# sonbui25/Multimodal-Aspect-Category-Sentiment-Analysis

Measured on AMD Instinct MI355X. Metric: train samples/sec (fwd+bwd+step) FCMF seq128x36ROI, higher is better.
Workload: dtype bf16; 1 GPU; FCMF-base fine-tune step, BASELINE configs[1]: batch 64 reviews x 6 aspects per GPU, seq 128, 7 images x (49 patches + 36 ROIs), precomputed ResNet-152 features, dropout 0.1, clip 1.0 + 4-group AdamW + linear schedule; global_batch=64, per_gpu_batch=64, seq_len=128, parallelism=dp1, sample_unit=1 review = 6 aspect forwards

## Files before the change

multimodal-aspect-category-sentiment-analysis_amd/csrc/misc.hip:

```cpp
#include "common.h"

template <typename T>
__global__ __launch_bounds__(256) void xent_fwd_kernel(const T* __restrict__ logits, int64_t ld,
                                                       const int64_t* __restrict__ labels, float* __restrict__ loss_rows,
                                                       float* __restrict__ nvalid, int n, int C, int64_t ignore_index) {
  const int lane = threadIdx.x & 63;
  const int row = blockIdx.x * 4 + (threadIdx.x >> 6);
  if (row >= n) return;
  const int64_t lab = labels[row];
  if (lab == ignore_index) { if (lane == 0) loss_rows[row] = 0.f; return; }
  const T* lr = logits + (int64_t)row * ld;
  float m = -INFINITY;
  for (int c = lane; c < C; c += 64) m = fmaxf(m, to_f32<T>(lr[c]));
  m = wave_max(m);
  float s = 0.f;
  for (int c = lane; c < C; c += 64) s += __expf(to_f32<T>(lr[c]) - m);
  s = wave_sum(s);
  if (lane == 0) {
    loss_rows[row] = (m + __logf(s)) - to_f32<T>(lr[lab]);
    if (nvalid) atomicAdd(nvalid, 1.0f);
  }
}

__global__ __launch_bounds__(256) void xent_mean_kernel(const float* __restrict__ loss_rows, const int64_t* __restrict__ labels,
                                                        int n, int64_t ignore_index, float mult, float* __restrict__ out2) {
  __shared__ double ssum[256];
  __shared__ int scnt[256];
  double s = 0.0;
  int c = 0;
  for (int i = threadIdx.x; i < n; i += 256)
    if (labels[i] != ignore_index) { s += (double)loss_rows[i]; ++c; }
  ssum[threadIdx.x] = s; scnt[threadIdx.x] = c;
  __syncthreads();
  for (int h = 128; h > 0; h >>= 1) {
    if ((int)threadIdx.x < h) { ssum[threadIdx.x] += ssum[threadIdx.x + h]; scnt[threadIdx.x] += scnt[threadIdx.x + h]; }
    __syncthreads();
  }
  if (threadIdx.x == 0) {
    const float nv = (float)scnt[0];
    out2[0] = mult * ((float)ssum[0] / nv);
    out2[1] = mult / nv;
  }
}

template <typename T>
__global__ __launch_bounds__(256) void bce_logits_kernel(const T* __restrict__ logits, int64_t ld, const float* __restrict__ target,
                                                         int64_t ldt, int n, int C, const float* __restrict__ dloss,
                                                         float* __restrict__ loss, T* __restrict__ dlogits, int64_t ldd,
                                                         float* __restrict__ probs) {
  __shared__ double ssum[256];
  const int64_t total = (int64_t)n * C;
  const float sc = (dloss ? *dloss : 1.0f) / (float)total;
  double s = 0.0;
// ... 102 lines not shown
  row_softmax_stats<T>(lr, C, vec != 0, m, s);
  if (threadIdx.x == 0) {
    loss_rows[row] = (m + __logf(s)) - to_f32<T>(lr[lab]);
    if (nvalid) atomicAdd(nvalid, 1.0f);
  }
}

template <typename T>
__global__ __launch_bounds__(256) void xent_bwd_wide_kernel(const T* logits, int64_t ld, const int64_t* __restrict__ labels,
                                                            T* dlogits, int64_t ldd, const float* __restrict__ scale_ptr,
                                                            float extra, int C, int64_t ignore_index, int vec) {
  constexpr int VN = XVec<T>::N;
  typedef typename XVec<T>::type vec_t;
  const int row = blockIdx.x, tid = threadIdx.x;
  const int64_t lab = labels[row];
  T* dr = dlogits + (int64_t)row * ldd;
  const int Cv = vec ? (C / VN) * VN : 0;
  if (lab == ignore_index) {
    vec_t z;
#pragma unroll
    for (int e = 0; e < VN; ++e) z[e] = from_f32<T>(0.f);
    for (int c = tid * VN; c < Cv; c += 256 * VN) *reinterpret_cast<vec_t*>(dr + c) = z;
    for (int c = Cv + tid; c < C; c += 256) dr[c] = from_f32<T>(0.f);
    return;
  }
  const T* lr = logits + (int64_t)row * ld;
  float m, s;
  row_softmax_stats<T>(lr, C, vec != 0, m, s);
  const float sc = (scale_ptr ? *scale_ptr : 1.0f) * extra, inv = sc / s;
  for (int c = tid * VN; c < Cv; c += 256 * VN) {
    const vec_t v = *reinterpret_cast<const vec_t*>(lr + c);
    vec_t o;
#pragma unroll
    for (int e = 0; e < VN; ++e) o[e] = from_f32<T>(__expf((float)v[e] - m) * inv - ((c + e) == lab ? sc : 0.f));
    *reinterpret_cast<vec_t*>(dr + c) = o;
  }
  for (int c = Cv + tid; c < C; c += 256) dr[c] = from_f32<T>(__expf(to_f32<T>(lr[c]) - m) * inv - (c == lab ? sc : 0.f));
}

template <typename TS, typename TD>
__global__ __launch_bounds__(256) void cast_kernel(const TS* __restrict__ s, TD* __restrict__ d, int64_t n) {
  const int64_t n4 = n >> 2;
  for (int64_t i = (int64_t)blockIdx.x * 256 + threadIdx.x; i < n4; i += (int64_t)gridDim.x * 256)
    Vec4<TD>::store(d + i * 4, Vec4<TS>::load(s + i * 4));
  if (blockIdx.x == 0 && threadIdx.x < (n & 3)) d[n4 * 4 + threadIdx.x] = from_f32<TD>(to_f32<TS>(s[n4 * 4 + threadIdx.x]));
}

template <typename TS, typename TD>
__global__ __launch_bounds__(256) void cast_unaligned_kernel(const TS* __restrict__ s, TD* __restrict__ d, int64_t n) {
  for (int64_t i = (int64_t)blockIdx.x * 256 + threadIdx.x; i < n; i += (int64_t)gridDim.x * 256)
    d[i] = from_f32<TD>(to_f32<TS>(s[i]));
}

__global__ __launch_bounds__(256) void cast_transpose_kernel(const float* __restrict__ src, bf16_t* __restrict__ dst, int R, int C) {
  __shared__ float tile[64][65];
  const int r0 = blockIdx.y * 64, c0 = blockIdx.x * 64;
  const int tx = threadIdx.x & 63, ty = threadIdx.x >> 6;
#pragma unroll
  for (int i = 0; i < 16; ++i) {
    const int r = r0 + ty * 16 + i, c = c0 + tx;
    tile[ty * 16 + i][tx] = (r < R && c < C) ? src[(int64_t)r * C + c] : 0.f;
  }
  __syncthreads();
  if ((R & 3) == 0) {
#pragma unroll
    for (int i = 0; i < 4; ++i) {
      const int cc = i * 16 + (threadIdx.x >> 4), rr = 4 * (threadIdx.x & 15);
      const int c = c0 + cc, r = r0 + rr;
      if (c < C && r < R) {
        bf16x4 o;
#pragma unroll
        for (int j = 0; j < 4; ++j) o[j] = (bf16_t)tile[rr + j][cc];
        *reinterpret_cast<bf16x4*>(dst + (int64_t)c * R + r) = o;
      }
    }
    return;
  }
#pragma unroll
  for (int i = 0; i < 16; ++i) {
    const int c = c0 + ty * 16 + i, r = r0 + tx;
    if (c < C && r < R) dst[(int64_t)c * R + r] = (bf16_t)tile[tx][ty * 16 + i];
  }
}

__global__ __launch_bounds__(256) void multi_cast_transpose_kernel(const int64_t* __restrict__ src_ptrs, const int64_t* __restrict__ dst_ptrs,
                                                                   const int32_t* __restrict__ dims, const int32_t* __restrict__ desc) {
  __shared__ float tile[64][65];
  const int t = desc[3 * blockIdx.x], r0 = desc[3 * blockIdx.x + 1] * 64, c0 = desc[3 * blockIdx.x + 2] * 64;
  const float* __restrict__ src = reinterpret_cast<const float*>(src_ptrs[t]);
  bf16_t* __restrict__ dst = reinterpret_cast<bf16_t*>(dst_ptrs[t]);
  const int R = dims[2 * t], C = dims[2 * t + 1];
  const int tx = threadIdx.x & 63, ty = threadIdx.x >> 6;
#pragma unroll
  for (int i = 0; i < 16; ++i) {
    const int r = r0 + ty * 16 + i, c = c0 + tx;
    tile[ty * 16 + i][tx] = (r < R && c < C) ? src[(int64_t)r * C + c] : 0.f;
  }
  __syncthreads();
#pragma unroll
  for (int i = 0; i < 16; ++i) {
    const int c = c0 + ty * 16 + i, r = r0 + tx;
    if (c < C && r < R) dst[(int64_t)c * R + r] = (bf16_t)tile[tx][ty * 16 + i];
  }
}

template <typename T>
__global__ __launch_bounds__(256) void dropout_kernel(const T* __restrict__ x, T* __restrict__ y, int64_t n, float p,
                                                      float inv_keep, uint64_t seed) {
  for (int64_t i = (int64_t)blockIdx.x * 256 + threadIdx.x; i < n; i += (int64_t)gridDim.x * 256)
    y[i] = from_f32<T>(to_f32<T>(x[i]) * dropout_mult(seed, (uint64_t)i, p, inv_keep));
}

template <typename T>
__global__ __launch_bounds__(256) void act_bwd_kernel(const T* __restrict__ dy, const T* __restrict__ aux, T* __restrict__ out,
                                                      int64_t n, int kind) {
  for (int64_t i = (int64_t)blockIdx.x * 256 + threadIdx.x; i < n; i += (int64_t)gridDim.x * 256) {
    const float a = to_f32<T>(aux[i]), d = to_f32<T>(dy[i]);
    out[i] = from_f32<T>(kind == 0 ? d * (1.0f - a * a) : d * dgelu_f(a));
  }
}

template <typename T>
__global__ __launch_bounds__(256) void sum_axis_kernel(const T* __restrict__ in, T* __restrict__ out, int64_t outer,
                                                       int reps, int64_t inner) {
  const int64_t total = outer * inner;
  for (int64_t i = (int64_t)blockIdx.x * 256 + threadIdx.x; i < total; i += (int64_t)gridDim.x * 256) {
    const int64_t o = i / inner, c = i - o * inner;
    float s = 0.f;
    for (int r = 0; r < reps; ++r) s += to_f32<T>(in[(o * reps + r) * inner + c]);
    out[i] = from_f32<T>(s);
  }
}

__global__ __launch_bounds__(256) void multi_sumsq_kernel(const int64_t* __restrict__ g_ptrs, const int64_t* __restrict__ sizes,
                                                          const int32_t* __restrict__ chunk_tensor,
                                                          const int64_t* __restrict__ chunk_offset, int chunk_size,
                                                          double* __restrict__ sumsq, double* __restrict__ per_tensor) {
  __shared__ double red[4];
  const int t = chunk_tensor[blockIdx.x];
  const int64_t off = chunk_offset[blockIdx.x];
  const float* g = reinterpret_cast<const float*>(g_ptrs[t]) + off;
  int64_t n = sizes[t] - off;
  if (n > chunk_size) n = chunk_size;
  double s = 0.0;
  const bool vec = (reinterpret_cast<uintptr_t>(g) & 15) == 0;
  if (vec) {
    const int64_t n4 = n >> 2;
    for (int64_t i = threadIdx.x; i < n4; i += 256) {
      const float4 v = *reinterpret_cast<const float4*>(g + i * 4);
      s += (double)v.x * v.x + (double)v.y * v.y + (double)v.z * v.z + (double)v.w * v.w;
    }
    for (int64_t i = n4 * 4 + threadIdx.x; i < n; i += 256) s += (double)g[i] * g[i];
  } else {
    for (int64_t i = threadIdx.x; i < n; i += 256) s += (double)g[i] * g[i];
  }
  s = wave_sum_d(s);
  if ((threadIdx.x & 63) == 0) red[threadIdx.x >> 6] = s;
  __syncthreads();
  if (threadIdx.x == 0) {
    const double tot = red[0] + red[1] + red[2] + red[3];
    if (sumsq) atomicAdd(sumsq, tot);
    if (per_tensor) atomicAdd(per_tensor + t, tot);
  }
}

struct AdamArgs {
  const int64_t *p_ptrs, *g_ptrs, *m_ptrs, *v_ptrs, *bf16_ptrs, *sizes;
  const int32_t *group_of, *chunk_tensor;
  const int64_t* chunk_offset;
  int chunk_size;
  float lr[8], wd[8];
  float beta1, beta2, eps, bc1, bc2_sqrt;
  const double* sumsq;
  float max_norm;
};

__global__ __launch_bounds__(256) void multi_adamw_kernel(AdamArgs a) {
#pragma clang fp contract(off)
  const int t = a.chunk_tensor[blockIdx.x];
  const int64_t off = a.chunk_offset[blockIdx.x];
  float* p = reinterpret_cast<float*>(a.p_ptrs[t]) + off;
  const float* g = reinterpret_cast<const float*>(a.g_ptrs[t]) + off;
  float* m = reinterpret_cast<float*>(a.m_ptrs[t]) + off;
  float* v = reinterpret_cast<float*>(a.v_ptrs[t]) + off;
  bf16_t* sh = a.bf16_ptrs && a.bf16_ptrs[t] ? reinterpret_cast<bf16_t*>(a.bf16_ptrs[t]) + off : nullptr;
  int64_t n = a.sizes[t] - off;
  if (n > a.chunk_size) n = a.chunk_size;
  const int grp = a.group_of[t];
  const float lr = a.lr[grp], wd = a.wd[grp];
  float coef = 1.0f;
  if (a.max_norm > 0.f && a.sumsq) {
    const float tn = (float)sqrt(*a.sumsq);
    coef = fminf(1.0f, a.max_norm / (tn + 1e-6f));
  }
  const float step_size = lr / a.bc1;
  typedef float f4 __attribute__((ext_vector_type(4)));
  int64_t i0 = 0;
  if (((reinterpret_cast<uintptr_t>(p) | reinterpret_cast<uintptr_t>(g) | reinterpret_cast<uintptr_t>(m) | reinterpret_cast<uintptr_t>(v)) & 15) == 0 &&
      (!sh || (reinterpret_cast<uintptr_t>(sh) & 7) == 0)) {
    const int64_t n4 = n >> 2;
    for (int64_t i = threadIdx.x; i < n4; i += 256) {
      const f4 g4 = __builtin_nontemporal_load(reinterpret_cast<const f4*>(g) + i) * coef;
      f4 p4 = reinterpret_cast<const f4*>(p)[i] * (1.0f - lr * wd);
// ... 5 lines not shown
      __builtin_nontemporal_store(m4, reinterpret_cast<f4*>(m) + i);
      __builtin_nontemporal_store(v4, reinterpret_cast<f4*>(v) + i);
      if (sh) {
        bf16x4 o;
        o[0] = (bf16_t)p4[0]; o[1] = (bf16_t)p4[1]; o[2] = (bf16_t)p4[2]; o[3] = (bf16_t)p4[3];
        reinterpret_cast<bf16x4*>(sh)[i] = o;
      }
    }
    i0 = n4 << 2;
  }
  for (int64_t i = i0 + threadIdx.x; i < n; i += 256) {
    const float gi = g[i] * coef;
    float pi = p[i] * (1.0f - lr * wd);
    const float mi = a.beta1 * m[i] + (1.0f - a.beta1) * gi;
    const float vi = a.beta2 * v[i] + (1.0f - a.beta2) * gi * gi;
    const float denom = sqrtf(vi) / a.bc2_sqrt + a.eps;
    pi -= step_size * (mi / denom);
    p[i] = pi; m[i] = mi; v[i] = vi;
    if (sh) sh[i] = (bf16_t)pi;
  }
}

__global__ __launch_bounds__(256) void sumsq_kernel(const float* __restrict__ g, int64_t n, double* __restrict__ out) {
  __shared__ double red[4];
  double s = 0.0;
  for (int64_t i = (int64_t)blockIdx.x * 256 + threadIdx.x; i < n; i += (int64_t)gridDim.x * 256) s += (double)g[i] * g[i];
  s = wave_sum_d(s);
  if ((threadIdx.x & 63) == 0) red[threadIdx.x >> 6] = s;
  __syncthreads();
  if (threadIdx.x == 0) atomicAdd(out, red[0] + red[1] + red[2] + red[3]);
}

__global__ __launch_bounds__(256) void bertadam_kernel(float* __restrict__ p, const float* __restrict__ g, float* __restrict__ m,
                                                       float* __restrict__ v, int64_t n, float lr, float b1, float b2, float e,
                                                       float wd, float max_norm, const double* __restrict__ sumsq) {
  float coef = 1.0f;
  if (max_norm > 0.f) coef = fminf(1.0f, max_norm / ((float)sqrt(*sumsq) + 1e-6f));
  for (int64_t i = (int64_t)blockIdx.x * 256 + threadIdx.x; i < n; i += (int64_t)gridDim.x * 256) {
    const float gi = g[i] * coef;
    const float mi = b1 * m[i] + (1.0f - b1) * gi;
    const float vi = b2 * v[i] + (1.0f - b2) * gi * gi;
    float upd = mi / (sqrtf(vi) + e);
    if (wd > 0.f) upd += wd * p[i];
    p[i] -= lr * upd;
    m[i] = mi; v[i] = vi;
  }
}

static int grid_for(int64_t n, int per) {
  int64_t b = (n + per - 1) / per;
  return (int)(b > 4096 ? 4096 : (b < 1 ? 1 : b));
}

extern "C" int fcmf_abi_version(void) { return 4; }
extern "C" const char* fcmf_build_info(void) { return "libfcmf_hip gfx950 (CDNA4, wave64) abi 4"; }

extern "C" int fcmf_xent_fwd(const void* logits, int64_t ld, const int64_t* labels, float* loss_rows, float* nvalid, int n,
                             int C, int64_t ignore_index, int dtype, void* stream) {
  if (!logits || !labels || !loss_rows || n < 0 || C <= 0) return FCMF_ERR_ARG;
  if (n == 0) return FCMF_OK;
  hipStream_t st = reinterpret_cast<hipStream_t>(stream);
  if (C >= 1024) {
    const int es = dtype == FCMF_F32 ? 4 : 2;
    const int vec = ((reinterpret_cast<uintptr_t>(logits) & 15) == 0) && ((ld * es) % 16 == 0);
    if (dtype == FCMF_F32) hipLaunchKernelGGL((xent_fwd_wide_kernel<float>), dim3(n), dim3(256), 0, st, (const float*)logits, ld, labels, loss_rows, nvalid, C, ignore_index, vec);
    else if (dtype == FCMF_BF16) hipLaunchKernelGGL((xent_fwd_wide_kernel<bf16_t>), dim3(n), dim3(256), 0, st, (const bf16_t*)logits, ld, labels, loss_rows, nvalid, C, ignore_index, vec);
    else return FCMF_ERR_UNSUPPORTED;
    FCMF_CHECK_LAUNCH();
    return FCMF_OK;
  }
  dim3 grid((n + 3) / 4);
  if (dtype == FCMF_F32) hipLaunchKernelGGL((xent_fwd_kernel<float>), grid, dim3(256), 0, st, (const float*)logits, ld, labels, loss_rows, nvalid, n, C, ignore_index);
  else if (dtype == FCMF_BF16) hipLaunchKernelGGL((xent_fwd_kernel<bf16_t>), grid, dim3(256), 0, st, (const bf16_t*)logits, ld, labels, loss_rows, nvalid, n, C, ignore_index);
  else return FCMF_ERR_UNSUPPORTED;
  FCMF_CHECK_LAUNCH();
  return FCMF_OK;
}

extern "C" int fcmf_xent_mean(const float* loss_rows, const int64_t* labels, int n, int64_t ignore_index, float mult,
                              float* out2, void* stream) {
  if (!loss_rows || !labels || !out2 || n < 0) return FCMF_ERR_ARG;
  hipLaunchKernelGGL(xent_mean_kernel, dim3(1), dim3(256), 0, reinterpret_cast<hipStream_t>(stream), loss_rows, labels, n,
                     ignore_index, mult, out2);
  FCMF_CHECK_LAUNCH();
  return FCMF_OK;
}

extern "C" int fcmf_bce_logits(const void* logits, int64_t ld, const float* target, int64_t ldt, int n, int C, const float* dloss,
                               float* loss, void* dlogits, int64_t ldd, float* probs, int dtype, void* stream) {
  if (!logits || (!target && (loss || dlogits)) || n < 0 || C <= 0 || ld < C || (target && ldt < C) || (dlogits && ldd < C))
    return FCMF_ERR_ARG;
  if (n == 0) return FCMF_OK;
  hipStream_t st = reinterpret_cast<hipStream_t>(stream);
  if (dtype == FCMF_F32)
    hipLaunchKernelGGL((bce_logits_kernel<float>), dim3(1), dim3(256), 0, st, (const float*)logits, ld, target, ldt, n, C, dloss, loss,
                       (float*)dlogits, ldd, probs);
  else if (dtype == FCMF_BF16)
    hipLaunchKernelGGL((bce_logits_kernel<bf16_t>), dim3(1), dim3(256), 0, st, (const bf16_t*)logits, ld, target, ldt, n, C, dloss, loss,
                       (bf16_t*)dlogits, ldd, probs);
  else return FCMF_ERR_UNSUPPORTED;
  FCMF_CHECK_LAUNCH();
  return FCMF_OK;
}

extern "C" int fcmf_additive_mask(const int64_t* mask, int64_t ld, float* out, int rows, int cols, float value, void* stream) {
  if (!mask || !out || rows < 0 || cols < 0 || ld < cols) return FCMF_ERR_ARG;
// ... 28 lines not shown
  FCMF_CHECK_LAUNCH();
  return FCMF_OK;
}

extern "C" int fcmf_cast(const void* src, void* dst, int64_t n, int src_dtype, int dst_dtype, void* stream) {
  if (!src || !dst || n < 0) return FCMF_ERR_ARG;
  if (n == 0) return FCMF_OK;
  hipStream_t st = reinterpret_cast<hipStream_t>(stream);
  if ((reinterpret_cast<uintptr_t>(src) & 15) || (reinterpret_cast<uintptr_t>(dst) & 7)) {
    const uintptr_t sm = src_dtype == FCMF_F32 ? 3 : 1, dm = dst_dtype == FCMF_F32 ? 3 : 1;
    if ((reinterpret_cast<uintptr_t>(src) & sm) || (reinterpret_cast<uintptr_t>(dst) & dm)) return FCMF_ERR_ARG;
    dim3 g1(grid_for(n, 256));
    if (src_dtype == FCMF_F32 && dst_dtype == FCMF_BF16) hipLaunchKernelGGL((cast_unaligned_kernel<float, bf16_t>), g1, dim3(256), 0, st, (const float*)src, (bf16_t*)dst, n);
    else if (src_dtype == FCMF_BF16 && dst_dtype == FCMF_F32) hipLaunchKernelGGL((cast_unaligned_kernel<bf16_t, float>), g1, dim3(256), 0, st, (const bf16_t*)src, (float*)dst, n);
    else if (src_dtype == FCMF_F32 && dst_dtype == FCMF_F32) hipLaunchKernelGGL((cast_unaligned_kernel<float, float>), g1, dim3(256), 0, st, (const float*)src, (float*)dst, n);
    else if (src_dtype == FCMF_BF16 && dst_dtype == FCMF_BF16) hipLaunchKernelGGL((cast_unaligned_kernel<bf16_t, bf16_t>), g1, dim3(256), 0, st, (const bf16_t*)src, (bf16_t*)dst, n);
    else return FCMF_ERR_UNSUPPORTED;
    FCMF_CHECK_LAUNCH();
    return FCMF_OK;
  }
  dim3 grid(grid_for(n, 1024));
  if (src_dtype == FCMF_F32 && dst_dtype == FCMF_BF16) hipLaunchKernelGGL((cast_kernel<float, bf16_t>), grid, dim3(256), 0, st, (const float*)src, (bf16_t*)dst, n);
  else if (src_dtype == FCMF_BF16 && dst_dtype == FCMF_F32) hipLaunchKernelGGL((cast_kernel<bf16_t, float>), grid, dim3(256), 0, st, (const bf16_t*)src, (float*)dst, n);
  else if (src_dtype == FCMF_F32 && dst_dtype == FCMF_F32) hipLaunchKernelGGL((cast_kernel<float, float>), grid, dim3(256), 0, st, (const float*)src, (float*)dst, n);
  else if (src_dtype == FCMF_BF16 && dst_dtype == FCMF_BF16) hipLaunchKernelGGL((cast_kernel<bf16_t, bf16_t>), grid, dim3(256), 0, st, (const bf16_t*)src, (bf16_t*)dst, n);
  else return FCMF_ERR_UNSUPPORTED;
  FCMF_CHECK_LAUNCH();
  return FCMF_OK;
}

extern "C" int fcmf_cast_transpose(const float* src, void* dst, int rows, int cols, void* stream) {
  if (!src || !dst || rows < 0 || cols < 0) return FCMF_ERR_ARG;
  if (rows == 0 || cols == 0) return FCMF_OK;
  dim3 grid((cols + 63) / 64, (rows + 63) / 64);
  hipLaunchKernelGGL(cast_transpose_kernel, grid, dim3(256), 0, reinterpret_cast<hipStream_t>(stream), src, (bf16_t*)dst, rows, cols);
  FCMF_CHECK_LAUNCH();
  return FCMF_OK;
}

extern "C" int fcmf_multi_cast_transpose(const int64_t* src_ptrs, const int64_t* dst_ptrs, const int32_t* dims,
                                         const int32_t* tile_desc, int ntiles, void* stream) {
  if (!src_ptrs || !dst_ptrs || !dims || !tile_desc || ntiles < 0) return FCMF_ERR_ARG;
  if (ntiles == 0) return FCMF_OK;
  hipLaunchKernelGGL(multi_cast_transpose_kernel, dim3(ntiles), dim3(256), 0, reinterpret_cast<hipStream_t>(stream), src_ptrs,
                     dst_ptrs, dims, tile_desc);
  FCMF_CHECK_LAUNCH();
  return FCMF_OK;
}

extern "C" int fcmf_dropout(const void* x, void* y, int64_t n, float p, uint64_t seed, int dtype, void* stream) {
  if (!x || !y || n < 0 || p < 0.f || p >= 1.f) return FCMF_ERR_ARG;
  if (n == 0) return FCMF_OK;
  hipStream_t st = reinterpret_cast<hipStream_t>(stream);
  dim3 grid(grid_for(n, 256));
  const float inv_keep = 1.0f / (1.0f - p);
  if (dtype == FCMF_F32) hipLaunchKernelGGL((dropout_kernel<float>), grid, dim3(256), 0, st, (const float*)x, (float*)y, n, p, inv_keep, seed);
  else if (dtype == FCMF_BF16) hipLaunchKernelGGL((dropout_kernel<bf16_t>), grid, dim3(256), 0, st, (const bf16_t*)x, (bf16_t*)y, n, p, inv_keep, seed);
  else return FCMF_ERR_UNSUPPORTED;
  FCMF_CHECK_LAUNCH();
  return FCMF_OK;
}

extern "C" int fcmf_act_bwd(const void* dy, const void* aux, void* out, int64_t n, int kind, int dtype, void* stream) {
  if (!dy || !aux || !out || n < 0 || (kind != 0 && kind != 1)) return FCMF_ERR_ARG;
  if (n == 0) return FCMF_OK;
  hipStream_t st = reinterpret_cast<hipStream_t>(stream);
  dim3 grid(grid_for(n, 256));
  if (dtype == FCMF_F32) hipLaunchKernelGGL((act_bwd_kernel<float>), grid, dim3(256), 0, st, (const float*)dy, (const float*)aux, (float*)out, n, kind);
  else if (dtype == FCMF_BF16) hipLaunchKernelGGL((act_bwd_kernel<bf16_t>), grid, dim3(256), 0, st, (const bf16_t*)dy, (const bf16_t*)aux, (bf16_t*)out, n, kind);
  else return FCMF_ERR_UNSUPPORTED;
  FCMF_CHECK_LAUNCH();
  return FCMF_OK;
}

template <typename T>
__global__ __launch_bounds__(256) void embed_scale_fwd_kernel(const int64_t* __restrict__ ids, const float* __restrict__ w,
                                                              const float* __restrict__ P, T* __restrict__ out, int n, int H,
                                                              int S, float scale, int64_t V) {
  const int lane = threadIdx.x & 63, row = blockIdx.x * 4 + (threadIdx.x >> 6);
  if (row >= n) return;
  const int64_t id = ids[row];
  if (id < 0 || id >= V) {
    const float q = __builtin_nanf("");
    for (int c = lane * 4; c < H; c += 256) Vec4<T>::store(out + (int64_t)row * H + c, make_float4(q, q, q, q));
    return;
  }
  const float* wr = w + id * (int64_t)H;
  const float* pr = P ? P + (int64_t)(row % S) * H : nullptr;
  for (int c = lane * 4; c < H; c += 256) {
    float4 v = *reinterpret_cast<const float4*>(wr + c);
    v.x *= scale; v.y *= scale; v.z *= scale; v.w *= scale;
    if (pr) {
      const float4 q = *reinterpret_cast<const float4*>(pr + c);
      v.x += q.x; v.y += q.y; v.z += q.z; v.w += q.w;
    }
    Vec4<T>::store(out + (int64_t)row * H + c, v);
  }
}
template <typename T>
__global__ __launch_bounds__(256) void embed_scale_bwd_kernel(const T* __restrict__ dy, const int64_t* __restrict__ ids,
                                                              float* __restrict__ dw, int n, int H, float scale, int64_t V,
                                                              int32_t* __restrict__ oob) {
  const int lane = threadIdx.x & 63, row = blockIdx.x * 4 + (threadIdx.x >> 6);
  if (row >= n) return;
  const int64_t id = ids[row];
  if (id < 0 || id >= V) {
    if (oob && lane == 0) atomicAdd(oob, 1);
    return;
  }
  float* wr = dw + id * (int64_t)H;
// ... 125 lines not shown
```

multimodal-aspect-category-sentiment-analysis_amd/csrc/norm.hip:

```cpp
#include "common.h"

constexpr int LN_MAXP = 8;

template <typename T, int NP>
__global__ __launch_bounds__(256) void add_ln_fwd_kernel(const T* __restrict__ x, const T* __restrict__ res,
                                                         int64_t res_stride, const float* __restrict__ gamma,
                                                         const float* __restrict__ beta, T* __restrict__ y,
                                                         T* __restrict__ z, float* __restrict__ mean,
                                                         float* __restrict__ rstd, int rows, int H, float eps,
                                                         float p, uint64_t seed, unsigned char* __restrict__ q8 = nullptr,
                                                         float* __restrict__ qscale = nullptr) {
  const int lane = threadIdx.x & 63;
  const float inv_keep = p > 0.f ? 1.0f / (1.0f - p) : 1.0f;
  typedef typename Vec4<T>::raw Raw;
  const int stride = gridDim.x * 4;
  int row = blockIdx.x * 4 + (threadIdx.x >> 6);
  Raw nx[NP], nr[NP];
  auto fetch = [&](int r) {
    if (r < rows) {
#pragma unroll
      for (int i = 0; i < NP; ++i) {
        const int c = (i * 64 + lane) * 4;
        if (c < H) {
          nx[i] = Vec4<T>::load_raw(x + (int64_t)r * H + c);
// ... 315 lines not shown
template <typename T>
__global__ __launch_bounds__(256) void embed_bwd_kernel(const T* __restrict__ dz, const int64_t* __restrict__ ids,
                                                        const int64_t* __restrict__ pos, const int64_t* __restrict__ tt,
                                                        float* __restrict__ dword, float* __restrict__ dpos,
                                                        float* __restrict__ dtt, int ntok, int H, int pad_id) {
  const int lane = threadIdx.x & 63;
  const int row = blockIdx.x * 4 + (threadIdx.x >> 6);
  if (row >= ntok) return;
  const int64_t id = ids[row], ps = pos[row], ty = tt ? tt[row] : 0;
  for (int c = lane; c < H; c += 64) {
    const float d = to_f32<T>(dz[(int64_t)row * H + c]);
    if (id != pad_id) atomicAdd(dword + id * H + c, d);
    if (dpos && ps != pad_id) atomicAdd(dpos + ps * H + c, d);
    if (dtt && ty != 0) atomicAdd(dtt + ty * H + c, d);
  }
}

template <typename T>
__global__ __launch_bounds__(256) void embed_type0_kernel(const T* __restrict__ dz, const int64_t* __restrict__ tt,
                                                          float* __restrict__ dtt, int ntok, int H, int rows_per_block) {
  __shared__ float red[4][64];
  const int lane = threadIdx.x & 63, w = threadIdx.x >> 6;
  const int col = blockIdx.x * 64 + lane;
  const int r0 = blockIdx.y * rows_per_block, r1 = min(ntok, r0 + rows_per_block);
  float s = 0.f;
  if (col < H)
    for (int r = r0 + w; r < r1; r += 4)
      if (!tt || tt[r] == 0) s += to_f32<T>(dz[(int64_t)r * H + col]);
  red[w][lane] = s;
  __syncthreads();
  if (w == 0 && col < H) atomicAdd(dtt + col, red[0][lane] + red[1][lane] + red[2][lane] + red[3][lane]);
}

template <typename T>
__global__ __launch_bounds__(256) void embed_pos_bwd_kernel(const T* __restrict__ dz, const int64_t* __restrict__ pos,
                                                            float* __restrict__ dpos, int nseq, int S, int H, int pad_id) {
  const int s = blockIdx.x, c = blockIdx.y * 256 + threadIdx.x;
  if (c >= H) return;
  int64_t p0 = -1;
  float acc = 0.f;
  const int g0 = blockIdx.z * 64, g1 = min(nseq, g0 + 64);
#pragma unroll 8
  for (int g = g0; g < g1; ++g) {
    const int64_t row = (int64_t)g * S + s, id = pos[row];
    if (id == pad_id) continue;
    const float d = to_f32<T>(dz[row * H + c]);
    if (p0 < 0) p0 = id;
    if (id == p0) acc += d;
    else atomicAdd(dpos + id * H + c, d);
  }
  if (p0 >= 0) atomicAdd(dpos + p0 * H + c, acc);
}

template <typename T>
__global__ __launch_bounds__(256) void embed_pos_type_bwd_kernel(const T* __restrict__ dz, const int64_t* __restrict__ pos,
                                                                 const int64_t* __restrict__ tt, float* __restrict__ dpos,
                                                                 float* __restrict__ dtt, int nseq, int S, int H, int pad_id) {
  constexpr int E = 16 / (int)sizeof(T);
  typedef T VecT __attribute__((ext_vector_type(E)));
  extern __shared__ __attribute__((aligned(16))) float red[];
  const int CE = H / E, slots = 256 / CE;
  const int tid = threadIdx.x, cg = tid % CE, slot = tid / CE, c0 = cg * E;
  const int s = blockIdx.x, g0 = blockIdx.y * 64, g1 = min(nseq, g0 + 64);
  float* rp = red;
  float* rt = red + slots * H;
  int* p0s = reinterpret_cast<int*>(red + 2 * slots * H);
  if (slot < slots) {
    float acc[E], tsum[E];
#pragma unroll
    for (int j = 0; j < E; ++j) acc[j] = tsum[j] = 0.f;
    int64_t p0 = -1;
#pragma unroll 4
    for (int g = g0 + slot; g < g1; g += slots) {
      const int64_t row = (int64_t)g * S + s, id = pos[row], ty = tt ? tt[row] : 0;
      const VecT v = *reinterpret_cast<const VecT*>(dz + row * H + c0);
      if (dtt) {
        if (ty == 0) {
#pragma unroll
          for (int j = 0; j < E; ++j) tsum[j] += (float)v[j];
        } else {
#pragma unroll
          for (int j = 0; j < E; ++j) atomicAdd(dtt + ty * H + c0 + j, (float)v[j]);
        }
      }
      if (id == pad_id) continue;
      if (p0 < 0) p0 = id;
      if (id == p0) {
#pragma unroll
        for (int j = 0; j < E; ++j) acc[j] += (float)v[j];
      } else {
#pragma unroll
        for (int j = 0; j < E; ++j) atomicAdd(dpos + id * H + c0 + j, (float)v[j]);
      }
    }
#pragma unroll
    for (int j = 0; j < E; ++j) { rp[slot * H + c0 + j] = acc[j]; rt[slot * H + c0 + j] = tsum[j]; }
    if (cg == 0) p0s[slot] = (int)p0;
  }
  __syncthreads();
  for (int c = tid; c < H; c += 256) {
    float ts = 0.f;
    for (int k = 0; k < slots; ++k) ts += rt[k * H + c];
    if (dtt) atomicAdd(dtt + c, ts);
    for (int k = 0; k < slots; ++k) {
      const int pk = p0s[k];
      if (pk < 0) continue;
      bool first = true;
      for (int m = 0; m < k; ++m) first = first && p0s[m] != pk;
      if (!first) continue;
      float ps = 0.f;
      for (int m = k; m < slots; ++m)
        if (p0s[m] == pk) ps += rp[m * H + c];
      atomicAdd(dpos + (int64_t)pk * H + c, ps);
    }
  }
}

#define LN_DISPATCH_T(T, H)                         \
  do {                                              \
    const int np__ = ((H) + 255) / 256;             \
    if (np__ <= 1) LAUNCH_(T, 1);                   \
    else if (np__ <= 2) LAUNCH_(T, 2);              \
    else if (np__ <= 3) LAUNCH_(T, 3);              \
    else if (np__ <= 4) LAUNCH_(T, 4);              \
    else LAUNCH_(T, 8);                             \
  } while (0)
#define LN_DISPATCH(dtype, H)                                     \
  do {                                                            \
    if ((dtype) == FCMF_F32) LN_DISPATCH_T(float, H);             \
    else LN_DISPATCH_T(bf16_t, H);                                \
  } while (0)

template <class K>
static int ln_resident_blocks(K kernel, int cap) {
  int dev = 0, cus = 0, per_cu = 0;
  if (hipGetDevice(&dev) != hipSuccess || hipDeviceGetAttribute(&cus, hipDeviceAttributeMultiprocessorCount, dev) != hipSuccess ||
      hipOccupancyMaxActiveBlocksPerMultiprocessor(&per_cu, kernel, 256, 0) != hipSuccess || cus <= 0 || per_cu <= 0) {
    (void)hipGetLastError();
    return cap;
  }
  return (int64_t)cus * per_cu < cap ? cus * per_cu : cap;
}

static int add_ln_fwd_impl(const void* x, const void* res, int64_t res_stride, const float* gamma, const float* beta, void* y,
                           void* z, float* mean, float* rstd, int rows, int H, float eps, float dropout_p, uint64_t seed,
                           int dtype, void* stream, void* q8, float* qscale);
extern "C" int fcmf_add_ln_fwd(const void* x, const void* res, int64_t res_stride, const float* gamma,
                               const float* beta, void* y, void* z, float* mean, float* rstd, int rows, int H,
                               float eps, float dropout_p, uint64_t seed, int dtype, void* stream) {
  return add_ln_fwd_impl(x, res, res_stride, gamma, beta, y, z, mean, rstd, rows, H, eps, dropout_p, seed, dtype, stream, nullptr, nullptr);
}
extern "C" int fcmf_add_ln_fwd_fp8(const void* x, const void* res, int64_t res_stride, const float* gamma,
                                   const float* beta, void* y, void* z, float* mean, float* rstd, int rows, int H,
                                   float eps, float dropout_p, uint64_t seed, int dtype, void* q8, float* qscale, void* stream) {
  if (!q8 || !qscale) return FCMF_ERR_ARG;
  return add_ln_fwd_impl(x, res, res_stride, gamma, beta, y, z, mean, rstd, rows, H, eps, dropout_p, seed, dtype, stream, q8, qscale);
}
static int add_ln_fwd_impl(const void* x, const void* res, int64_t res_stride, const float* gamma, const float* beta, void* y,
                           void* z, float* mean, float* rstd, int rows, int H, float eps, float dropout_p, uint64_t seed,
                           int dtype, void* stream, void* q8, float* qscale) {
  if (!x || !gamma || !beta || !y || !mean || !rstd || rows < 0 || H <= 0) return FCMF_ERR_ARG;
  if (H % 4 != 0 || H > LN_MAXP * 256 || (res && res_stride % 4 != 0)) return FCMF_ERR_UNSUPPORTED;
  if (rows == 0) return FCMF_OK;
  hipStream_t st = reinterpret_cast<hipStream_t>(stream);
  const int nblk = (rows + 3) / 4;
// ... 62 lines not shown
  if (!ids || !pos || nseq < 0 || S <= 0) return FCMF_ERR_ARG;
  if (nseq == 0) return FCMF_OK;
  hipLaunchKernelGGL(position_ids_kernel, dim3(nseq), dim3(64), 0, reinterpret_cast<hipStream_t>(stream), ids, pos, S, pad_id);
  FCMF_CHECK_LAUNCH();
  return FCMF_OK;
}

extern "C" int fcmf_embed_ln_fwd(const int64_t* ids, const int64_t* pos, const int64_t* type_ids, const float* word,
                                 const float* pos_table, const float* type_table, const float* gamma, const float* beta,
                                 void* y, void* z, float* mean, float* rstd, int ntok, int H, float eps, float dropout_p,
                                 uint64_t seed, int dtype, void* stream) {
  if (!ids || !pos || !word || !pos_table || !type_table || !gamma || !beta || !y || !mean || !rstd) return FCMF_ERR_ARG;
  if (H % 4 != 0 || H > LN_MAXP * 256) return FCMF_ERR_UNSUPPORTED;
  if (ntok <= 0) return ntok == 0 ? FCMF_OK : FCMF_ERR_ARG;
  hipStream_t st = reinterpret_cast<hipStream_t>(stream);
  dim3 grid((ntok + 3) / 4);
  if (dtype != FCMF_F32 && dtype != FCMF_BF16) return FCMF_ERR_UNSUPPORTED;
#define LAUNCH_(T, NP) hipLaunchKernelGGL((embed_ln_fwd_kernel<T, NP>), grid, dim3(256), 0, st, ids, pos, type_ids, word, \
    pos_table, type_table, gamma, beta, (T*)y, (T*)z, mean, rstd, ntok, H, eps, dropout_p, seed)
  LN_DISPATCH(dtype, H);
#undef LAUNCH_
  FCMF_CHECK_LAUNCH();
  return FCMF_OK;
}

extern "C" int fcmf_embed_bwd(const void* dz, const int64_t* ids, const int64_t* pos, const int64_t* type_ids, float* dword,
                              float* dpos, float* dtype_table, int ntok, int H, int pad_id, int dtype, void* stream) {
  if (!dz || !ids || !pos || !dword) return FCMF_ERR_ARG;
  if (H % 4 != 0) return FCMF_ERR_UNSUPPORTED;
  if (ntok <= 0) return ntok == 0 ? FCMF_OK : FCMF_ERR_ARG;
  hipStream_t st = reinterpret_cast<hipStream_t>(stream);
  dim3 grid((ntok + 3) / 4);
  const int rpb = 512;
  dim3 g2((H + 63) / 64, (ntok + rpb - 1) / rpb);
  if (dtype == FCMF_F32) {
    hipLaunchKernelGGL((embed_bwd_kernel<float>), grid, dim3(256), 0, st, (const float*)dz, ids, pos, type_ids, dword, dpos, dtype_table, ntok, H, pad_id);
    if (dtype_table) hipLaunchKernelGGL((embed_type0_kernel<float>), g2, dim3(256), 0, st, (const float*)dz, type_ids, dtype_table, ntok, H, rpb);
  } else if (dtype == FCMF_BF16) {
    hipLaunchKernelGGL((embed_bwd_kernel<bf16_t>), grid, dim3(256), 0, st, (const bf16_t*)dz, ids, pos, type_ids, dword, dpos, dtype_table, ntok, H, pad_id);
    if (dtype_table) hipLaunchKernelGGL((embed_type0_kernel<bf16_t>), g2, dim3(256), 0, st, (const bf16_t*)dz, type_ids, dtype_table, ntok, H, rpb);
  } else return FCMF_ERR_UNSUPPORTED;
  FCMF_CHECK_LAUNCH();
  return FCMF_OK;
}

extern "C" int fcmf_embed_pos_type_bwd(const void* dz, const int64_t* pos, const int64_t* type_ids, float* dpos, float* dtype_table,
                                       int nseq, int S, int H, int pad_id, int dtype, void* stream) {
  if (!dz || !pos || !dpos || nseq < 0 || S <= 0 || H <= 0) return FCMF_ERR_ARG;
  if (nseq == 0) return FCMF_OK;
  if (dtype != FCMF_F32 && dtype != FCMF_BF16) return FCMF_ERR_UNSUPPORTED;
  const int E = dtype == FCMF_F32 ? 4 : 8;
  if (H % E != 0 || H / E > 256 || (reinterpret_cast<uintptr_t>(dz) & 15)) return FCMF_ERR_UNSUPPORTED;
  hipStream_t st = reinterpret_cast<hipStream_t>(stream);
  const int slots = 256 / (H / E);
  const size_t smem = sizeof(float) * 2 * (size_t)slots * H + sizeof(int) * slots;
  dim3 grid(S, (nseq + 63) / 64);
  if (dtype == FCMF_F32) hipLaunchKernelGGL((embed_pos_type_bwd_kernel<float>), grid, dim3(256), smem, st, (const float*)dz, pos, type_ids, dpos, dtype_table, nseq, S, H, pad_id);
  else hipLaunchKernelGGL((embed_pos_type_bwd_kernel<bf16_t>), grid, dim3(256), smem, st, (const bf16_t*)dz, pos, type_ids, dpos, dtype_table, nseq, S, H, pad_id);
  FCMF_CHECK_LAUNCH();
  return FCMF_OK;
}

extern "C" int fcmf_embed_pos_bwd(const void* dz, const int64_t* pos, float* dpos, int nseq, int S, int H, int pad_id,
                                  int dtype, void* stream) {
  if (!dz || !pos || !dpos || nseq < 0 || S <= 0 || H <= 0) return FCMF_ERR_ARG;
  if (nseq == 0) return FCMF_OK;
  hipStream_t st = reinterpret_cast<hipStream_t>(stream);
  dim3 grid(S, (H + 255) / 256, (nseq + 63) / 64);
  if (dtype == FCMF_F32) hipLaunchKernelGGL((embed_pos_bwd_kernel<float>), grid, dim3(256), 0, st, (const float*)dz, pos, dpos, nseq, S, H, pad_id);
  else if (dtype == FCMF_BF16) hipLaunchKernelGGL((embed_pos_bwd_kernel<bf16_t>), grid, dim3(256), 0, st, (const bf16_t*)dz, pos, dpos, nseq, S, H, pad_id);
  else return FCMF_ERR_UNSUPPORTED;
  FCMF_CHECK_LAUNCH();
  return FCMF_OK;
}
```

Baseline: 1836 samples/s.

## Vectorize and batch loads in cast-transpose, dropout, sumsq and pos/type embedding backward

The cast-transpose tile now loads the source with 16-byte vector reads when alignment allows. Dropout becomes a vectorized streaming kernel that batches several loads per thread, handles unaligned head and tail elements, and uses a smaller grid. The grad-norm sumsq kernel unrolls eight vector loads per iteration, and the pos/type embedding backward splits the hidden dimension into column blocks and sets sequences per block to expose more parallelism and memory-level overlap. The goal is better bandwidth in these memory-bound auxiliary kernels, at the cost of more complex code and changed edge handling.

Measured after the change: 1841 samples/s, median of 6. No clear change (+0.3%).

```diff
diff --git a/multimodal-aspect-category-sentiment-analysis_amd/csrc/misc.hip b/multimodal-aspect-category-sentiment-analysis_amd/csrc/misc.hip
--- a/multimodal-aspect-category-sentiment-analysis_amd/csrc/misc.hip
+++ b/multimodal-aspect-category-sentiment-analysis_amd/csrc/misc.hip
@@ -1,4 +1,7 @@
 #include "common.h"
+
+template <typename T>
+__device__ __forceinline__ T* global_ptr(int64_t addr) { return (T*)reinterpret_cast<__attribute__((address_space(1))) T*>(addr); }
 
 template <typename T>
 __global__ __launch_bounds__(256) void xent_fwd_kernel(const T* __restrict__ logits, int64_t ld,
@@ -207,17 +210,28 @@
     d[i] = from_f32<TD>(to_f32<TS>(s[i]));
 }
 
-__global__ __launch_bounds__(256) void cast_transpose_kernel(const float* __restrict__ src, bf16_t* __restrict__ dst, int R, int C) {
-  __shared__ float tile[64][65];
-  const int r0 = blockIdx.y * 64, c0 = blockIdx.x * 64;
+__device__ __forceinline__ void cast_transpose_tile(const float* __restrict__ src, bf16_t* __restrict__ dst, int R, int C, int r0, int c0,
+                                                    float (&tile)[64][65]) {
   const int tx = threadIdx.x & 63, ty = threadIdx.x >> 6;
-#pragma unroll
-  for (int i = 0; i < 16; ++i) {
-    const int r = r0 + ty * 16 + i, c = c0 + tx;
-    tile[ty * 16 + i][tx] = (r < R && c < C) ? src[(int64_t)r * C + c] : 0.f;
+  if ((C & 3) == 0 && C > 0 && R > 0 && (reinterpret_cast<uintptr_t>(src) & 15) == 0) {
+    const int rr = threadIdx.x >> 4, cc = 4 * (threadIdx.x & 15);
+    const int c = min(c0 + cc, C - 4);
+    f32x4 v[4];
+#pragma unroll
+    for (int i = 0; i < 4; ++i) v[i] = *reinterpret_cast<const f32x4*>(src + (int64_t)min(r0 + i * 16 + rr, R - 1) * C + c);
+#pragma unroll
+    for (int i = 0; i < 4; ++i)
+#pragma unroll
+      for (int j = 0; j < 4; ++j) tile[i * 16 + rr][cc + j] = v[i][j];
+  } else {
+#pragma unroll
+    for (int i = 0; i < 16; ++i) {
+      const int r = r0 + ty * 16 + i, c = c0 + tx;
+      tile[ty * 16 + i][tx] = (r < R && c < C) ? src[(int64_t)r * C + c] : 0.f;
+    }
   }
   __syncthreads();
-  if ((R & 3) == 0) {
+  if ((R & 3) == 0 && (reinterpret_cast<uintptr_t>(dst) & 7) == 0) {
 #pragma unroll
     for (int i = 0; i < 4; ++i) {
       const int cc = i * 16 + (threadIdx.x >> 4), rr = 4 * (threadIdx.x & 15);
@@ -238,32 +252,73 @@
   }
 }
 
+__global__ __launch_bounds__(256) void cast_transpose_kernel(const float* __restrict__ src, bf16_t* __restrict__ dst, int R, int C) {
+  __shared__ float tile[64][65];
+  cast_transpose_tile(src, dst, R, C, blockIdx.y * 64, blockIdx.x * 64, tile);
+}
+
 __global__ __launch_bounds__(256) void multi_cast_transpose_kernel(const int64_t* __restrict__ src_ptrs, const int64_t* __restrict__ dst_ptrs,
                                                                    const int32_t* __restrict__ dims, const int32_t* __restrict__ desc) {
   __shared__ float tile[64][65];
-  const int t = desc[3 * blockIdx.x], r0 = desc[3 * blockIdx.x + 1] * 64, c0 = desc[3 * blockIdx.x + 2] * 64;
-  const float* __restrict__ src = reinterpret_cast<const float*>(src_ptrs[t]);
-  bf16_t* __restrict__ dst = reinterpret_cast<bf16_t*>(dst_ptrs[t]);
-  const int R = dims[2 * t], C = dims[2 * t + 1];
-  const int tx = threadIdx.x & 63, ty = threadIdx.x >> 6;
-#pragma unroll
-  for (int i = 0; i < 16; ++i) {
-    const int r = r0 + ty * 16 + i, c = c0 + tx;
-    tile[ty * 16 + i][tx] = (r < R && c < C) ? src[(int64_t)r * C + c] : 0.f;
-  }
-  __syncthreads();
-#pragma unroll
-  for (int i = 0; i < 16; ++i) {
-    const int c = c0 + ty * 16 + i, r = r0 + tx;
-    if (c < C && r < R) dst[(int64_t)c * R + r] = (bf16_t)tile[tx][ty * 16 + i];
-  }
-}
-
-template <typename T>
-__global__ __launch_bounds__(256) void dropout_kernel(const T* __restrict__ x, T* __restrict__ y, int64_t n, float p,
+  const int t = desc[3 * blockIdx.x];
+  cast_transpose_tile(global_ptr<const float>(src_ptrs[t]), global_ptr<bf16_t>(dst_ptrs[t]), dims[2 * t], dims[2 * t + 1],
+                      desc[3 * blockIdx.x + 1] * 64, desc[3 * blockIdx.x + 2] * 64, tile);
+}
+
+constexpr int STREAM_U = 4, STREAM_MAX_BLOCKS = 2048;
+
+template <typename T> struct Stream {
+  static constexpr int E = 16 / (int)sizeof(T);
+  typedef T vec __attribute__((ext_vector_type(E)));
+};
+
+template <class Load, class Use>
+__device__ __forceinline__ void stream_batches(int64_t nv, Load load, Use use) {
+  typedef decltype(load((int64_t)0)) V;
+  const int64_t nth = (int64_t)gridDim.x * 256;
+  int64_t i = (int64_t)blockIdx.x * 256 + threadIdx.x;
+  V v[STREAM_U];
+  for (; i + (STREAM_U - 1) * nth < nv; i += STREAM_U * nth) {
+#pragma unroll
+    for (int u = 0; u < STREAM_U; ++u) v[u] = load(i + u * nth);
+#pragma unroll
+    for (int u = 0; u < STREAM_U; ++u) use(i + u * nth, v[u]);
+  }
+#pragma unroll
+  for (int u = 0; u < STREAM_U; ++u) {
+    v[u] = V{};
+    if (i + u * nth < nv) v[u] = load(i + u * nth);
+  }
+#pragma unroll
+  for (int u = 0; u < STREAM_U; ++u)
+    if (i + u * nth < nv) use(i + u * nth, v[u]);
+}
+template <class Scalar>
+__device__ __forceinline__ void stream_edges(int64_t n, int64_t head, int64_t nv, int E, Scalar scalar) {
+  const int64_t tail0 = head + nv * E, edges = head + (n - tail0);
+  for (int64_t i = (int64_t)blockIdx.x * 256 + threadIdx.x; i < edges; i += (int64_t)gridDim.x * 256)
+    scalar(i < head ? i : tail0 + (i - head));
+}
+
+template <typename T>
+__global__ __launch_bounds__(256) void dropout_kernel(const T* __restrict__ x, T* __restrict__ y, int64_t n, int64_t head, float p,
                                                       float inv_keep, uint64_t seed) {
-  for (int64_t i = (int64_t)blockIdx.x * 256 + threadIdx.x; i < n; i += (int64_t)gridDim.x * 256)
-    y[i] = from_f32<T>(to_f32<T>(x[i]) * dropout_mult(seed, (uint64_t)i, p, inv_keep));
+  constexpr int E = Stream<T>::E;
+  typedef typename Stream<T>::vec vec;
+  const int64_t nv = (n - head) / E;
+  stream_batches(nv, [&](int64_t i) { return *reinterpret_cast<const vec*>(x + head + i * E); },
+                 [&](int64_t i, vec v) {
+                   vec o;
+#pragma unroll
+                   for (int q = 0; q < E; q += 4) {
+                     float m[4];
+                     dropout_mult4(seed, (uint64_t)(head + i * E + q), p, inv_keep, m);
+#pragma unroll
+                     for (int j = 0; j < 4; ++j) o[q + j] = from_f32<T>(to_f32<T>(v[q + j]) * m[j]);
+                   }
+                   *reinterpret_cast<vec*>(y + head + i * E) = o;
+                 });
+  stream_edges(n, head, nv, E, [&](int64_t i) { y[i] = from_f32<T>(to_f32<T>(x[i]) * dropout_mult(seed, (uint64_t)i, p, inv_keep)); });
 }
 
 template <typename T>
@@ -287,6 +342,7 @@
   }
 }
 
+constexpr int SUMSQ_U = 8;
 __global__ __launch_bounds__(256) void multi_sumsq_kernel(const int64_t* __restrict__ g_ptrs, const int64_t* __restrict__ sizes,
                                                           const int32_t* __restrict__ chunk_tensor,
                                                           const int64_t* __restrict__ chunk_offset, int chunk_size,
@@ -294,16 +350,33 @@
   __shared__ double red[4];
   const int t = chunk_tensor[blockIdx.x];
   const int64_t off = chunk_offset[blockIdx.x];
-  const float* g = reinterpret_cast<const float*>(g_ptrs[t]) + off;
+  const float* g = global_ptr<const float>(g_ptrs[t]) + off;
   int64_t n = sizes[t] - off;
   if (n > chunk_size) n = chunk_size;
   double s = 0.0;
   const bool vec = (reinterpret_cast<uintptr_t>(g) & 15) == 0;
   if (vec) {
     const int64_t n4 = n >> 2;
-    for (int64_t i = threadIdx.x; i < n4; i += 256) {
-      const float4 v = *reinterpret_cast<const float4*>(g + i * 4);
-      s += (double)v.x * v.x + (double)v.y * v.y + (double)v.z * v.z + (double)v.w * v.w;
+    const f32x4* g4 = reinterpret_cast<const f32x4*>(g);
+    f32x4 v[SUMSQ_U];
+    auto add = [&]() {
+#pragma unroll
+      for (int u = 0; u < SUMSQ_U; ++u)
+        s += (double)v[u][0] * v[u][0] + (double)v[u][1] * v[u][1] + (double)v[u][2] * v[u][2] + (double)v[u][3] * v[u][3];
+    };
+    int64_t i = threadIdx.x;
+    for (; i + (SUMSQ_U - 1) * 256 < n4; i += SUMSQ_U * 256) {
+#pragma unroll
+      for (int u = 0; u < SUMSQ_U; ++u) v[u] = g4[i + u * 256];
+      add();
+    }
+    if (i < n4) {
+#pragma unroll
+      for (int u = 0; u < SUMSQ_U; ++u) {
+        v[u] = f32x4{0.f, 0.f, 0.f, 0.f};
+        if (i + u * 256 < n4) v[u] = g4[i + u * 256];
+      }
+      add();
     }
     for (int64_t i = n4 * 4 + threadIdx.x; i < n; i += 256) s += (double)g[i] * g[i];
   } else {
@@ -415,6 +488,19 @@
   return (int)(b > 4096 ? 4096 : (b < 1 ? 1 : b));
 }
 
+static int64_t stream_head(int64_t n, int es, const void* a, const void* b) {
+  const uintptr_t oa = reinterpret_cast<uintptr_t>(a) & 15, ob = reinterpret_cast<uintptr_t>(b) & 15;
+  if (oa != ob || oa % es) return n;
+  const int64_t head = oa ? (int64_t)(16 - oa) / es : 0;
+  return head < n ? head : n;
+}
+static int stream_grid(int64_t n, int64_t head, int es) {
+  const int64_t nv = (n - head) / (16 / es), edges = n - nv * (16 / es);
+  int64_t b = (nv + 256 * STREAM_U - 1) / (256 * STREAM_U);
+  if (b < (edges + 255) / 256) b = (edges + 255) / 256;
+  return (int)(b > STREAM_MAX_BLOCKS ? STREAM_MAX_BLOCKS : (b < 1 ? 1 : b));
+}
+
 extern "C" int fcmf_abi_version(void) { return 4; }
 extern "C" const char* fcmf_build_info(void) { return "libfcmf_hip gfx950 (CDNA4, wave64) abi 4"; }
 
@@ -549,10 +635,13 @@
   if (!x || !y || n < 0 || p < 0.f || p >= 1.f) return FCMF_ERR_ARG;
   if (n == 0) return FCMF_OK;
   hipStream_t st = reinterpret_cast<hipStream_t>(stream);
-  dim3 grid(grid_for(n, 256));
+  if (dtype != FCMF_F32 && dtype != FCMF_BF16) return FCMF_ERR_UNSUPPORTED;
+  const int es = dtype == FCMF_F32 ? 4 : 2;
+  const int64_t head = stream_head(n, es, x, y);
+  dim3 grid(stream_grid(n, head, es));
   const float inv_keep = 1.0f / (1.0f - p);
-  if (dtype == FCMF_F32) hipLaunchKernelGGL((dropout_kernel<float>), grid, dim3(256), 0, st, (const float*)x, (float*)y, n, p, inv_keep, seed);
-  else if (dtype == FCMF_BF16) hipLaunchKernelGGL((dropout_kernel<bf16_t>), grid, dim3(256), 0, st, (const bf16_t*)x, (bf16_t*)y, n, p, inv_keep, seed);
+  if (dtype == FCMF_F32) hipLaunchKernelGGL((dropout_kernel<float>), grid, dim3(256), 0, st, (const float*)x, (float*)y, n, head, p, inv_keep, seed);
+  else if (dtype == FCMF_BF16) hipLaunchKernelGGL((dropout_kernel<bf16_t>), grid, dim3(256), 0, st, (const bf16_t*)x, (bf16_t*)y, n, head, p, inv_keep, seed);
   else return FCMF_ERR_UNSUPPORTED;
   FCMF_CHECK_LAUNCH();
   return FCMF_OK;
diff --git a/multimodal-aspect-category-sentiment-analysis_amd/csrc/norm.hip b/multimodal-aspect-category-sentiment-analysis_amd/csrc/norm.hip
--- a/multimodal-aspect-category-sentiment-analysis_amd/csrc/norm.hip
+++ b/multimodal-aspect-category-sentiment-analysis_amd/csrc/norm.hip
@@ -391,28 +391,46 @@
   if (p0 >= 0) atomicAdd(dpos + p0 * H + c, acc);
 }
 
+constexpr int PTB_U = 8, PTB_CB = 32;
 template <typename T>
 __global__ __launch_bounds__(256) void embed_pos_type_bwd_kernel(const T* __restrict__ dz, const int64_t* __restrict__ pos,
                                                                  const int64_t* __restrict__ tt, float* __restrict__ dpos,
-                                                                 float* __restrict__ dtt, int nseq, int S, int H, int pad_id) {
+                                                                 float* __restrict__ dtt, int nseq, int S, int H, int pad_id,
+                                                                 int seq_per_block) {
   constexpr int E = 16 / (int)sizeof(T);
   typedef T VecT __attribute__((ext_vector_type(E)));
   extern __shared__ __attribute__((aligned(16))) float red[];
-  const int CE = H / E, slots = 256 / CE;
-  const int tid = threadIdx.x, cg = tid % CE, slot = tid / CE, c0 = cg * E;
-  const int s = blockIdx.x, g0 = blockIdx.y * 64, g1 = min(nseq, g0 + 64);
+  const int CB = min(H / E, PTB_CB), slots = 256 / CB, CBW = CB * E;
+  const int tid = threadIdx.x, cg = tid % CB, slot = tid / CB;
+  const int cb0 = blockIdx.y * CBW, c0 = cb0 + cg * E;
+  const int s = blockIdx.x, g0 = blockIdx.z * seq_per_block, g1 = min(nseq, g0 + seq_per_block);
   float* rp = red;
-  float* rt = red + slots * H;
-  int* p0s = reinterpret_cast<int*>(red + 2 * slots * H);
+  float* rt = red + slots * CBW;
+  int* p0s = reinterpret_cast<int*>(red + 2 * slots * CBW);
   if (slot < slots) {
     float acc[E], tsum[E];
 #pragma unroll
     for (int j = 0; j < E; ++j) acc[j] = tsum[j] = 0.f;
     int64_t p0 = -1;
-#pragma unroll 4
-    for (int g = g0 + slot; g < g1; g += slots) {
-      const int64_t row = (int64_t)g * S + s, id = pos[row], ty = tt ? tt[row] : 0;
-      const VecT v = *reinterpret_cast<const VecT*>(dz + row * H + c0);
+    if (c0 < H) {
+    for (int gb = g0 + slot; gb < g1; gb += PTB_U * slots) {
+    VecT vb[PTB_U];
+    int64_t idb[PTB_U], tyb[PTB_U];
+#pragma unroll
+    for (int u = 0; u < PTB_U; ++u) {
+      const int g = gb + u * slots;
+      vb[u] = VecT{}; idb[u] = pad_id; tyb[u] = 0;
+      if (g < g1) {
+        const int64_t row = (int64_t)g * S + s;
+        idb[u] = pos[row]; tyb[u] = tt ? tt[row] : 0;
+        vb[u] = *reinterpret_cast<const VecT*>(dz + row * H + c0);
+      }
+    }
+#pragma unroll
+    for (int u = 0; u < PTB_U; ++u) {
+      if (gb + u * slots >= g1) break;
+      const int64_t id = idb[u], ty = tyb[u];
+      const VecT v = vb[u];
       if (dtt) {
         if (ty == 0) {
 #pragma unroll
@@ -432,14 +450,17 @@
         for (int j = 0; j < E; ++j) atomicAdd(dpos + id * H + c0 + j, (float)v[j]);
       }
     }
-#pragma unroll
-    for (int j = 0; j < E; ++j) { rp[slot * H + c0 + j] = acc[j]; rt[slot * H + c0 + j] = tsum[j]; }
+    }
+    }
+#pragma unroll
+    for (int j = 0; j < E; ++j) { rp[slot * CBW + cg * E + j] = acc[j]; rt[slot * CBW + cg * E + j] = tsum[j]; }
     if (cg == 0) p0s[slot] = (int)p0;
   }
   __syncthreads();
-  for (int c = tid; c < H; c += 256) {
+  for (int lc = tid; lc < CBW && cb0 + lc < H; lc += 256) {
+    const int c = cb0 + lc;
     float ts = 0.f;
-    for (int k = 0; k < slots; ++k) ts += rt[k * H + c];
+    for (int k = 0; k < slots; ++k) ts += rt[k * CBW + lc];
     if (dtt) atomicAdd(dtt + c, ts);
     for (int k = 0; k < slots; ++k) {
       const int pk = p0s[k];
@@ -449,7 +470,7 @@
       if (!first) continue;
       float ps = 0.f;
       for (int m = k; m < slots; ++m)
-        if (p0s[m] == pk) ps += rp[m * H + c];
+        if (p0s[m] == pk) ps += rp[m * CBW + lc];
       atomicAdd(dpos + (int64_t)pk * H + c, ps);
     }
   }
@@ -618,11 +639,14 @@
   const int E = dtype == FCMF_F32 ? 4 : 8;
   if (H % E != 0 || H / E > 256 || (reinterpret_cast<uintptr_t>(dz) & 15)) return FCMF_ERR_UNSUPPORTED;
   hipStream_t st = reinterpret_cast<hipStream_t>(stream);
-  const int slots = 256 / (H / E);
-  const size_t smem = sizeof(float) * 2 * (size_t)slots * H + sizeof(int) * slots;
-  dim3 grid(S, (nseq + 63) / 64);
-  if (dtype == FCMF_F32) hipLaunchKernelGGL((embed_pos_type_bwd_kernel<float>), grid, dim3(256), smem, st, (const float*)dz, pos, type_ids, dpos, dtype_table, nseq, S, H, pad_id);
-  else hipLaunchKernelGGL((embed_pos_type_bwd_kernel<bf16_t>), grid, dim3(256), smem, st, (const bf16_t*)dz, pos, type_ids, dpos, dtype_table, nseq, S, H, pad_id);
+  const int CE = H / E, CB = CE < PTB_CB ? CE : PTB_CB, slots = 256 / CB, ncb = (CE + CB - 1) / CB;
+  const size_t smem = sizeof(float) * 2 * (size_t)slots * CB * E + sizeof(int) * slots;
+  int groups = 256 / (int)((int64_t)S * ncb > 256 ? 256 : (int64_t)S * ncb);
+  if (groups > (nseq + 63) / 64) groups = (nseq + 63) / 64;
+  const int spb = (nseq + groups - 1) / groups;
+  dim3 grid(S, ncb, (nseq + spb - 1) / spb);
+  if (dtype == FCMF_F32) hipLaunchKernelGGL((embed_pos_type_bwd_kernel<float>), grid, dim3(256), smem, st, (const float*)dz, pos, type_ids, dpos, dtype_table, nseq, S, H, pad_id, spb);
+  else hipLaunchKernelGGL((embed_pos_type_bwd_kernel<bf16_t>), grid, dim3(256), smem, st, (const bf16_t*)dz, pos, type_ids, dpos, dtype_table, nseq, S, H, pad_id, spb);
   FCMF_CHECK_LAUNCH();
   return FCMF_OK;
 }
```
